# peter-seres/python-ray-tracer

Measured on AMD Instinct MI355X. Metric: Mrays/sec + frame time (ms) at 1920x1080, 8 spheres, depth=3, higher is better.
Workload: dtype f64

## Files before the change

### python-ray-tracer_amd/csrc/rt_device.h

```cpp
#pragma once
#include <hip/hip_runtime.h>
#include <stdint.h>

#pragma clang fp contract(off)

#ifndef RT_FAST_DIVSQRT
#define RT_FAST_DIVSQRT 1
#endif
#ifndef RT_FAST_NORMALIZE
#define RT_FAST_NORMALIZE 1
#endif
#ifndef RT_W_PARK
#define RT_W_PARK 7
#endif
#ifndef RT_W_AAPARK
#define RT_W_AAPARK 7
#endif
#ifndef RT_W_LANES
#define RT_W_LANES 4
#endif

namespace rt {

constexpr int TILE = 8;
// ... 151 lines not shown

enum { HIT_NONE = 0, HIT_SPHERE = 1, HIT_PLANE = 2 };

typedef __attribute__((address_space(3))) double lds_f64;
__device__ __forceinline__ unsigned fresh_lane()
{
    unsigned l;
    asm volatile("v_mbcnt_lo_u32_b32 %0, -1, 0\n\tv_mbcnt_hi_u32_b32 %0, -1, %0" : "=v"(l));
    return l;
}
template <bool PARK, int WGT, bool REMAT = false> struct Park3 {
    volatile lds_f64 *p;
    volatile lds_f64 *sbase;
    V3 v;
    __device__ __forceinline__ Park3(double *base, int slot, int wave = 0)
        : p(REMAT ? nullptr : (volatile lds_f64 *)base + slot * 3 * WGT + threadIdx.x),
          sbase(REMAT ? (volatile lds_f64 *)base + slot * 3 * WGT + wave * 64 : nullptr), v{0.0, 0.0, 0.0} {}
    __device__ __forceinline__ volatile lds_f64 *at() const { if constexpr (REMAT) return sbase + fresh_lane(); else return p; }
    __device__ __forceinline__ void set(const V3 &a)
    {
        if constexpr (PARK) { volatile lds_f64 *q = at(); q[0] = a.x; q[WGT] = a.y; q[2 * WGT] = a.z; } else v = a;
    }
    __device__ __forceinline__ V3 get() const
    {
        if constexpr (PARK) { volatile lds_f64 *q = at(); return V3{q[0], q[WGT], q[2 * WGT]}; } else return v;
    }
};

enum class Family { PLAIN, MAT, REFR, SCAT, SOFT, LENS, LENS_SOFT };
constexpr int FAMILIES = 7;
__host__ __device__ constexpr bool has_mat(Family f) { return f != Family::PLAIN; }
__host__ __device__ constexpr bool has_refr(Family f) { return f >= Family::REFR; }
__host__ __device__ constexpr bool has_scat(Family f) { return f >= Family::SCAT; }
__host__ __device__ constexpr bool has_soft(Family f) { return f == Family::SOFT || f == Family::LENS_SOFT; }
__host__ __device__ constexpr bool has_lens(Family f) { return f >= Family::LENS; }
__host__ __device__ constexpr int table_cols(Family f) { return has_scat(f) ? 6 : (has_refr(f) ? 5 : 3); }

template <Family F, int WSLOT, bool FRESH> struct MatState {
    static constexpr bool mat = true, refr = has_refr(F), scat = has_scat(F), soft = has_soft(F), lens = has_lens(F);
    static constexpr int COLS = table_cols(F);
    unsigned tab;
    unsigned ids;
    int nsh;
    enum { W = 0, LAMB = 1, REFL = 2, QX = 3, QY = 4, QZ = 5, ETA = 6, ROUGH = 7, KEY = 8, LKEY = 9 };
    template <int WGT, int k> __device__ __forceinline__ volatile lds_f64 *at(const double *acc, int wave) const
    {
        if constexpr (FRESH) return (volatile lds_f64 *)acc + (WSLOT + k) * WGT + wave * 64 + fresh_lane();
        else return (volatile lds_f64 *)acc + (WSLOT + k) * WGT + threadIdx.x;
    }
    __device__ __forceinline__ volatile const lds_f64 *entry(int slot) const
    {
        unsigned t = tab, i = ids;
        asm volatile("" : "+s"(t), "+s"(i));
        typedef __attribute__((address_space(3))) const int lds_ci32;
        const int m = ((lds_ci32 *)(size_t)i)[slot];
        return (volatile const lds_f64 *)(size_t)t + COLS * m;
    }
};
template <int WSLOT, bool FRESH> struct MatState<Family::PLAIN, WSLOT, FRESH> {
    static constexpr bool mat = false, refr = false, scat = false, soft = false, lens = false;
};

constexpr float CULL_K_ANCHOR = 0x1p-19f * 1.0001f;
constexpr float CULL_K_ORIGIN = 0x1p-18f;
constexpr float CULL_K_S = 0x1p-21f;
constexpr float CULL_K_FLOOR = 0x1p-40f;

extern __shared__ double lds_raw[];

struct Lds {
    __device__ __forceinline__ const double *recs() const { return lds_raw; }
    const float *sph32;
    const float *tab;
    const float *csph32;
    const float *ctab;
    const float *cbox;
    const float *gbox;
    const float *gtab;
    const float *col32;
    int NC;
    int wave;
    bool pairs;
    bool groups;
#ifdef RT_REGION_STATS
    unsigned *reg;
#endif
    double *acc;
};

#ifdef RT_REGION_STATS
__device__ __forceinline__ void region_mark(unsigned *reg, int id)
{
    volatile unsigned *r = reg + (threadIdx.x >> 6) * 32;
    const unsigned now = (unsigned)__builtin_amdgcn_s_memtime();
    const unsigned last = r[31], c = r[30];
    r[id + c] = r[id + c] + (now - last);
    r[31] = now;
}
#define RT_MARK(id) region_mark(lds.reg, id)
#else
#define RT_MARK(id)
#endif

struct RayF {
    F3 o, R;
    float mgq, esq;
};

__device__ __forceinline__ RayF make_rayf_dir(const V3 &R)
{
    RayF q;
    q.o = F3{0.0f, 0.0f, 0.0f};
    q.R = F3{(float)R.x, (float)R.y, (float)R.z};
    q.mgq = 0.0f; q.esq = 0.0f;
    return q;
}
__device__ __forceinline__ void add_origin(RayF &q, const V3 &o, float extent2)
{
    q.o = F3{(float)o.x, (float)o.y, (float)o.z};
    const float oo = __builtin_fmaf(q.o.z, q.o.z, __builtin_fmaf(q.o.y, q.o.y, q.o.x * q.o.x));
    q.mgq = __builtin_fmaf(CULL_K_ORIGIN, oo, CULL_K_FLOOR * (oo + extent2));
    q.esq = __builtin_fmaf(CULL_K_S, oo, CULL_K_S);
}

__device__ __forceinline__ float anchored_tau(double ll, double r2, float floor_anch)
{
    const double W = ((ll - r2) - (ll + r2) * (double)CULL_K_ANCHOR) - (double)floor_anch;
    if (!(W > 0.0)) return 0.0f;
    return (float)(__builtin_sqrt(W) * (1.0 - 0x1p-20));
}

typedef float f4 __attribute__((ext_vector_type(4)));
typedef __attribute__((address_space(3))) const f4 lds_cf4;
__device__ __forceinline__ lds_cf4 *pin_lds(const float *generic)
{
    unsigned a = (unsigned)(size_t)(__attribute__((address_space(3))) const float *)generic;
    asm volatile("" : "+v"(a));
    return (lds_cf4 *)(size_t)a;
}

__device__ __forceinline__ bool cull_anchored(const f4 e, const RayF &q)
{
    const float s = __builtin_fmaf(e[2], q.R.z, __builtin_fmaf(e[1], q.R.y, e[0] * q.R.x));
    return __builtin_fabsf(s) < e[3];
}

__device__ __forceinline__ bool cull_origin(const f4 c, const RayF &q)
{
    const float lx = q.o.x - c[0], ly = q.o.y - c[1], lz = q.o.z - c[2];
    const float s = __builtin_fmaf(lz, q.R.z, __builtin_fmaf(ly, q.R.y, lx * q.R.x));
    const float ll = __builtin_fmaf(lz, lz, __builtin_fmaf(ly, ly, lx * lx));
    const float cc = ll - c[3];
    const float D = __builtin_fmaf(s, s, -cc);
    const float mg = __builtin_fmaf(CULL_K_ORIGIN, ll + c[3], q.mgq);
    const float es = __builtin_fmaf(CULL_K_S, ll, q.esq);
    return (bool)((int)(D < -mg) | ((int)(s > es) & (int)(cc > mg)));
}

typedef unsigned long long lanemask;
__device__ __forceinline__ lanemask m_nlt_abs(float a, float b)
{
    lanemask m; asm volatile("v_cmp_nlt_f32_e64 %0, |%1|, %2" : "=s"(m) : "v"(a), "v"(b)); return m;
}
__device__ __forceinline__ lanemask m_nlt_neg(float a, float b)
{
    lanemask m; asm volatile("v_cmp_nlt_f32_e64 %0, %1, -%2" : "=s"(m) : "v"(a), "v"(b)); return m;
// ... 85 lines not shown
            open = m_nlt_abs(sd, e[3]);
        } else {
            const float lx = q.o.x - e[0], ly = q.o.y - e[1], lz = q.o.z - e[2];
            const float sd = __builtin_fmaf(lz, q.R.z, __builtin_fmaf(ly, q.R.y, lx * q.R.x));
            const float ll = __builtin_fmaf(lz, lz, __builtin_fmaf(ly, ly, lx * lx));
            const float cc = ll - e[3];
            const float D = __builtin_fmaf(sd, sd, -cc);
            const float mg = __builtin_fmaf(CULL_K_ORIGIN, ll + e[3], q.mgq);
            const float es = __builtin_fmaf(CULL_K_S, ll, q.esq);
            open = m_nlt_neg(D, mg) & (m_ngt(sd, es) | m_ngt(cc, mg));
        }
        if constexpr (SELF) open &= m_ne(jsel, u);
        acc = push_any(acc, open);
    }
    return acc;
}

template <bool ANCH, bool SELF>
__device__ __forceinline__ unsigned long long cull_mask_t(const Lds &lds, int S, int anchor, int k0, int n,
                                                          const RayF &q, int selfj)
{
    unsigned long long mask = 0ull;
    const int Sp = padS(S, lds.NC);
    lds_cf4 *sbase = pin_lds(ANCH ? lds.tab + ((size_t)anchor * Sp + k0) * CULL_STRIDE : lds.sph32 + 4 * k0);
    if (lds.NC > 0) {
        const int NCp = pad4(lds.NC), c0 = k0 / CLUSTER, nc = (n + CLUSTER - 1) / CLUSTER;
        if (ANCH && lds.groups) {
            static_assert(CLUSTER * SUPER == 64, "a 64-sphere chunk is one group of clusters");
            const f4 ge = *pin_lds(lds.gtab + ((size_t)anchor * pad4(supers(lds.NC)) + (k0 >> 6)) * CULL_STRIDE);
            const float gs = __builtin_fmaf(ge[2], q.R.z, __builtin_fmaf(ge[1], q.R.y, ge[0] * q.R.x));
            if (m_nlt_abs(gs, ge[3]) == 0ull) return 0ull;
        }
        lds_cf4 *cbase = pin_lds(ANCH ? lds.ctab + ((size_t)anchor * NCp + c0) * CULL_STRIDE : lds.csph32 + 4 * c0);
        unsigned cm = 0;
        for (int j = 0; j < nc; j += 4) cm |= (lds.pairs ? cull4<ANCH, false, true>(cbase + j, q, -1, 0u) : cull4<ANCH, false, false>(cbase + j, q, -1, 0u)) << j;
        while (cm) {
            const int c = __builtin_ctz(cm);
            cm &= cm - 1u;
            const int jb = c * CLUSTER;
            const unsigned hi = lds.pairs ? cull4<ANCH, SELF, true>(sbase + jb + 4, q, selfj - jb - 4, 0u) : cull4<ANCH, SELF, false>(sbase + jb + 4, q, selfj - jb - 4, 0u);
            const unsigned lohi = lds.pairs ? cull4<ANCH, SELF, true>(sbase + jb, q, selfj - jb, hi) : cull4<ANCH, SELF, false>(sbase + jb, q, selfj - jb, hi);
            mask |= (unsigned long long)lohi << jb;
        }
    } else {
        const int npad = pad4(n);
        for (int j = 0; j < npad; j += 4) mask |= (unsigned long long)(lds.pairs ? cull4<ANCH, SELF, true>(sbase + j, q, selfj - j, 0u) : cull4<ANCH, SELF, false>(sbase + j, q, selfj - j, 0u)) << j;
    }
    return mask;
}

__device__ __forceinline__ unsigned long long cull_mask(const Lds &lds, int S, int anchor, int k0, int n,
                                                        const V3 &o, const V3 &R, float extent2, int self)
{
    RayF q = make_rayf_dir(R);
    if (anchor >= 0) {
        const bool cand = self >= k0 && self < k0 + n;
        if (__builtin_amdgcn_ballot_w64(cand) != 0ull) {
            add_origin(q, o, extent2);
            const float *cs = lds.sph32 + 4 * self;
            const bool self_culled = cand ? cull_origin(f4{cs[0], cs[1], cs[2], cs[3]}, q) : false;
            if (__builtin_amdgcn_ballot_w64(self_culled) != 0ull)
                return cull_mask_t<true, true>(lds, S, anchor, k0, n, q, self_culled ? self - k0 : -1);
        }
        return cull_mask_t<true, false>(lds, S, anchor, k0, n, q, -1);
    }
    add_origin(q, o, extent2);
    return cull_mask_t<false, false>(lds, S, anchor, k0, n, q, -1);
}


__device__ __forceinline__ int opaque(int x)
{
    asm volatile("" : "+s"(x));
    return x;
}

__device__ __forceinline__ int plane_code(const KParams &p, int k)
{
    unsigned c = p.plane_codes;
    asm volatile("" : "+s"(c));
    return k < 4 ? (int)(signed char)(c >> (8 * k)) : 0;
}

__device__ __forceinline__ void plane_den_num(const double *__restrict__ g, int code, const V3 &o, const V3 &d, double &den, double &num)
{
    if (code == 0) {
        const V3 n{g[3], g[4], g[5]};
        den = dot3(d, n);
        const V3 LP{g[0] - o.x, g[1] - o.y, g[2] - o.z};
        num = dot3(LP, n);
    } else {
        const int a = code < 0 ? -code : code;
        double dc, lp;
        if (a == 1)      { dc = d.x; lp = g[0] - o.x; }
        else if (a == 2) { dc = d.y; lp = g[1] - o.y; }
        else             { dc = d.z; lp = g[2] - o.z; }
        if (code > 0) { den = dc; num = lp; } else { den = -dc; num = -lp; }
    }
}

struct SphHot { double x, y, z, r2; };
template <bool F32> __device__ __forceinline__ SphHot sphere_hot(const Lds &lds, int k)
{
    if constexpr (F32) {
        const f4 c = *(lds_cf4 *)(size_t)(unsigned)(size_t)(__attribute__((address_space(3))) const float *)(lds.sph32 + 4 * k);
        return SphHot{(double)c[0], (double)c[1], (double)c[2], (double)c[3]};
    } else {
        const double *g = lds.recs() + k * SPH_STRIDE;
        return SphHot{g[0], g[1], g[2], g[3]};
    }
}
template <bool F32> __device__ __forceinline__ double sphere_orig(const Lds &lds, const KParams &p, int k)
{
    if constexpr (F32) return p.scene[(size_t)k * SPH_STRIDE + 7]; else return lds.recs()[k * SPH_STRIDE + 7];
}

template <bool F32>
__device__ __forceinline__ void sphere_closest(const Lds &lds, const KParams &p, int k, const V3 &o, const V3 &R, double a,
                                               double &bestn, int &bidx)
{
    const SphHot g = sphere_hot<F32>(lds, k);
    const V3 Lv{o.x - g.x, o.y - g.y, o.z - g.z};
    const double s = dot3(Lv, R);
    const double cc = dot3(Lv, Lv) - g.r2;
    const double D = s * s - a * cc;
    if (D >= 0.0 && !(s >= 0.0 && cc >= 0.0)) {
        const double q = sqrt_inrange(D);
        double n = -s - q;
        if (!(n > 0.0)) n = -s + q;
        if (n > 0.0) {
            bool take = n < bestn;
            const bool close = __builtin_fabs(n - bestn) < bestn * 0x1p-50;
            if (__builtin_amdgcn_ballot_w64(close) != 0ull) {
                if (close) {
                    const double tq = n / a, tb = bestn / a;
                    take = tq < tb || (tq == tb && sphere_orig<F32>(lds, p, k) < sphere_orig<F32>(lds, p, bidx));
                }
            }
            if (take) { bestn = n; bidx = k; }
        }
    }
}

template <bool F32>
__device__ __forceinline__ bool sphere_any(const Lds &lds, int k, const V3 &o, const V3 &R, double a, bool a_sane)
{
    const SphHot g = sphere_hot<F32>(lds, k);
    const V3 Lv{o.x - g.x, o.y - g.y, o.z - g.z};
    const double s = dot3(Lv, R);
    const double cc = dot3(Lv, Lv) - g.r2;
    const double D = s * s - a * cc;
    if (D >= 0.0 && !(s >= 0.0 && cc >= 0.0)) {
        if (s < 0.0 && -s < 499.0 && D < 249001.0 && a_sane) return true;
        const double q = __builtin_sqrt(D);
        double n = -s - q;
        if (!(n > 0.0)) n = -s + q;
        if (n > 0.0) {
            const double t = n / a;
            if (999.0 > t && t > 0.0) return true;
        }
    }
    return false;
}


template <bool ANCH>
__device__ __forceinline__ bool lane_open(const f4 e, const RayF &q)
{
    if constexpr (ANCH) {
        const float sd = __builtin_fmaf(e[2], q.R.z, __builtin_fmaf(e[1], q.R.y, e[0] * q.R.x));
        return !(__builtin_fabsf(sd) < e[3]);
    } else return !cull_origin(e, q);
}
__device__ __forceinline__ lds_cf4 *lds_f4(const float *generic)
{
    return (lds_cf4 *)(size_t)(unsigned)(size_t)(__attribute__((address_space(3))) const float *)generic;
}

template <bool ANCH>
__device__ __forceinline__ unsigned lane_cluster_bits(const Lds &lds, int anchor, int cb, int nc, const RayF &q, float extent2)
{
    unsigned cm = 0u;
    if constexpr (ANCH) {
        const int NCp = pad4(lds.NC), NGp = pad4(supers(lds.NC));
        lds_cf4 *base = pin_lds(lds.ctab + ((size_t)anchor * NCp + cb) * CULL_STRIDE);
        lds_cf4 *gbase = pin_lds(lds.gtab + ((size_t)anchor * NGp + cb / SUPER) * CULL_STRIDE);
        for (int c0 = 0; c0 < nc; c0 += SUPER) {
            if (__builtin_amdgcn_ballot_w64(lane_open<true>(gbase[c0 / SUPER], q)) == 0ull) continue;
            const int c1 = c0 + SUPER < nc ? c0 + SUPER : nc;
            for (int c = c0; c < c1; c += 4) {
#pragma unroll
                for (int u = 0; u < 4; ++u) {
                    asm volatile("" ::: "memory");
                    const f4 e = base[c + u];
                    cm |= lane_open<true>(e, q) ? (1u << (c + u)) : 0u;
                }
            }
        }
    } else {
        const RayBox rb = make_raybox(q, extent2);
        lds_cf4 *base = pin_lds(lds.cbox + (size_t)cb * BOX_STRIDE);
        lds_cf4 *gbase = pin_lds(lds.gbox + (size_t)(cb / SUPER) * BOX_STRIDE);
        static_assert(SUPER == 8, "a group's clusters are one byte of the mask");
        for (int c0 = 0; c0 < nc; c0 += SUPER) {
            const bool gopen = box_open(gbase[2 * (c0 / SUPER)], gbase[2 * (c0 / SUPER) + 1], rb) || !rb.sane;
            if (__builtin_amdgcn_ballot_w64(gopen) == 0ull) continue;
            const int c1 = c0 + SUPER < nc ? c0 + SUPER : nc;
            for (int c = c0; c < c1; c += 2) {
#pragma unroll
                for (int u = 0; u < 2; ++u) {
                    asm volatile("" ::: "memory");
                    const f4 lo = base[2 * (c + u)], hi = base[2 * (c + u) + 1];
                    cm |= box_open(lo, hi, rb) ? (1u << (c + u)) : 0u;
                }
            }
        }
        if (!rb.sane) cm = ~0u;
    }
    return cm & (nc >= 32 ? ~0u : ((1u << nc) - 1u));
}

template <bool ANCH>
__device__ __forceinline__ unsigned lane_sphere_bits(const Lds &lds, int S, int anchor, int kb, const RayF &q)
{
    const int Sp = padS(S, lds.NC);
    lds_cf4 *sb = lds_f4(ANCH ? lds.tab + ((size_t)anchor * Sp + kb) * CULL_STRIDE : lds.sph32 + 4 * kb);
    unsigned sm = 0u;
#pragma unroll
    for (int j = 0; j < CLUSTER; ++j) sm |= lane_open<ANCH>(sb[j], q) ? (1u << j) : 0u;
    const int nv = S - kb;
    return nv >= CLUSTER ? sm : (sm & ((1u << nv) - 1u));
}

#ifdef RT_LANE_STATS
__device__ __forceinline__ void lane_stats(const KParams &p, int base, unsigned v)
{
    if (!p.tile_cycles) return;
    unsigned mx = v, sum = v;
    for (int d = 32; d >= 1; d >>= 1) { const unsigned m2 = __shfl_xor(mx, d), s2 = __shfl_xor(sum, d); mx = m2 > mx ? m2 : mx; sum += s2; }
    if ((threadIdx.x & 63) == __builtin_ctzll(__builtin_amdgcn_ballot_w64(true))) {
        unsigned *c = p.tile_cycles + p.ntiles + base;
        atomicAdd(c + 0, 1u); atomicAdd(c + 1, mx); atomicAdd(c + 2, (sum + 63u) >> 6); atomicAdd(c + 3, sum);
    }
}
#endif
// ... 47 lines not shown
        if (__builtin_amdgcn_ballot_w64(self >= 0) != 0ull) {
            add_origin(q, o, p.extent2);
            if (self >= 0) { const float *cs = lds.sph32 + 4 * self; self_culled = cull_origin(f4{cs[0], cs[1], cs[2], cs[3]}, q); }
        }
    } else add_origin(q, o, p.extent2);
    bool occ = false;
    for (int cb = 0; cb < lds.NC; cb += 32) {
        if (cb > 0 && __builtin_amdgcn_ballot_w64(!occ) == 0ull) break;
        const int nc = lds.NC - cb < 32 ? lds.NC - cb : 32;
        unsigned cm = lane_cluster_bits<ANCH>(lds, anchor, cb, nc, q, p.extent2);
        RT_MARK(7);
        if (occ) cm = 0u;
#ifdef RT_LANE_STATS
        lane_stats(p, 8, __builtin_popcount(cm));
#endif
        while (__builtin_amdgcn_ballot_w64(cm != 0u) != 0ull) {
#ifdef RT_LANE_STATS
            unsigned smc = 0;
#endif
            if (cm != 0u) {
                const int kb = (cb + __builtin_ctz(cm)) * CLUSTER;
                cm &= cm - 1u;
                unsigned sm = lane_sphere_bits<ANCH>(lds, p.S, anchor, kb, q);
                if (self_culled && self >= kb && self < kb + CLUSTER) sm &= ~(1u << (self - kb));
#ifdef RT_LANE_STATS
                smc = __builtin_popcount(sm);
#endif
                while (__builtin_amdgcn_ballot_w64(sm != 0u) != 0ull) {
                    if (sm != 0u) {
                        const int k = kb + __builtin_ctz(sm);
                        sm &= sm - 1u;
                        if (sphere_any<true>(lds, k, o, R, a, a_sane)) { occ = true; sm = 0u; cm = 0u; }
                    }
                }
            }
#ifdef RT_LANE_STATS
            lane_stats(p, 12, smc);
#endif
        }
        RT_MARK(8);
    }
    return occ;
}

template <int MODE>
__device__ __forceinline__ void closest_hit(const Lds &lds, const KParams &p, const V3 &o, const V3 &d, int anchor,
                                            double &t_out, int &idx_out, int &type_out)
{
    const int P = opaque(p.P);
    const int S = p.S;
    const V3 R = renormalize_unit(d);
    const double a = dot3(R, R);
    RT_MARK(0);
    const int canchor = (opaque(p.anchors) > 0) ? anchor : -1;
    double bestn = __builtin_inf();
    int bidx = -1;
    constexpr bool F32 = MODE >= 1;
    if (MODE >= 2 && lds.NC > 0 && (canchor < 0 || p.lanes_primary)) {
        if (canchor >= 0) lanes_closest<true>(lds, p, canchor, o, R, a, bestn, bidx);
        else lanes_closest<false>(lds, p, -1, o, R, a, bestn, bidx);
    } else
    for (int k0 = 0; k0 < S; k0 += 64) {
      const int n = (S - k0 < 64) ? S - k0 : 64;
      unsigned long long mask = cull_mask(lds, S, canchor, k0, n, o, R, p.extent2, -1);
      mask &= (n == 64) ? ~0ull : ((1ull << n) - 1ull);
      RT_MARK(1);
      while (mask) {
        const int k = k0 + __builtin_ctzll(mask);
        mask &= mask - 1ull;
        sphere_closest<F32>(lds, p, k, o, R, a, bestn, bidx);
      }
      RT_MARK(2);
    }
    double best = 999.0;
    int idx = -1, type = HIT_NONE;
    if (bidx >= 0) {
        const double t = div_inrange(bestn, a);
        if (best > t && t > 0.0) { best = t; idx = bidx; type = HIT_SPHERE; }
    }
    const double *pl = lds.recs() + (F32 ? 0 : opaque(p.S) * SPH_STRIDE);
    for (int k = 0; k < P; ++k) {
        const double *g = pl + k * PL_STRIDE;
        double den, num;
        plane_den_num(g, plane_code(p, k), o, d, den, num);
        if (!(__builtin_fabs(den) < 0.001)) {
            const double t = div_inrange(num, den);
            if (best > t && t > 0.0) { best = t; idx = k; type = HIT_PLANE; }
        }
    }
    t_out = best; idx_out = idx; type_out = type;
    RT_MARK(3);
}

template <int MODE>
__device__ __forceinline__ bool any_hit(const Lds &lds, const KParams &p, const V3 &o, const V3 &d, int anchor, int self, bool lanes = true)
{
    const int P = opaque(p.P);
    const int S = p.S;
    const V3 R = renormalize_unit(d);
    const double a = dot3(R, R);
    RT_MARK(6);
    const bool a_sane = (a > 0.999999 && a < 1.000001);
    bool occ = false;
    const int canchor = (opaque(p.anchors) > 0) ? anchor : -1;
    if (MODE >= 2 && lds.NC > 0 && lanes) {
        occ = (canchor >= 0) ? lanes_any<true>(lds, p, canchor, o, R, a, self) : lanes_any<false>(lds, p, -1, o, R, a, self);
    } else
    for (int k0 = 0; k0 < S; k0 += 64) {
      if (k0 > 0 && __builtin_amdgcn_ballot_w64(!occ) == 0ull) break;
      const int n = (S - k0 < 64) ? S - k0 : 64;
      unsigned long long mask = cull_mask(lds, S, canchor, k0, n, o, R, p.extent2, self);
      mask &= (n == 64) ? ~0ull : ((1ull << n) - 1ull);
      RT_MARK(7);
      while (mask) {
        const int k = k0 + __builtin_ctzll(mask);
        mask &= mask - 1ull;
        if (!occ) occ = sphere_any<(MODE >= 1)>(lds, k, o, R, a, a_sane);
        if (mask && __builtin_amdgcn_ballot_w64(!occ) == 0ull) break;
      }
      RT_MARK(8);
    }
    const double *pl = lds.recs() + (MODE >= 1 ? 0 : opaque(p.S) * SPH_STRIDE);
    for (int k = 0; k < P; ++k) {
        if (!occ) {
            const double *g = pl + k * PL_STRIDE;
            double den, num;
            plane_den_num(g, plane_code(p, k), o, d, den, num);
            if (!(__builtin_fabs(den) < 0.001)) {
                const double an = __builtin_fabs(num), ad = __builtin_fabs(den);
                const bool same_sign = (num > 0.0 && den > 0.0) || (num < 0.0 && den < 0.0);
                if (same_sign) {
                    if (an < 998.0 * ad) occ = true;
                    else if (!(an > 1000.0 * ad)) { const double t = num / den; if (999.0 > t && t > 0.0) occ = true; }
                }
            }
        }
    }
    RT_MARK(9);
    return occ;
}

template <bool COUNT> struct RayCount {
    __device__ __forceinline__ void closest(bool) {}
    __device__ __forceinline__ void hit(bool) {}
    __device__ __forceinline__ void shadow(bool, bool) {}
};
template <> struct RayCount<true> {
    unsigned n_closest = 0, n_issued = 0, n_skipped = 0, n_hit = 0;
    __device__ __forceinline__ void closest(bool alive) { n_closest += alive ? 1u : 0u; }
    __device__ __forceinline__ void hit(bool alive) { n_hit += alive ? 1u : 0u; }
    __device__ __forceinline__ void shadow(bool alive, bool traced) { n_issued += (alive && traced) ? 1u : 0u; n_skipped += (alive && !traced) ? 1u : 0u; }
};

__device__ __forceinline__ unsigned scatter_key(unsigned x, unsigned y, unsigned s, unsigned seed)
{
    unsigned h = (seed ^ 0x5CA77E12u) ^ 0x9E3779B9u;
    h = (h ^ x) * 0x85EBCA6Bu; h ^= h >> 13;
    h = (h ^ y) * 0xC2B2AE35u; h ^= h >> 16;
    return h ^ (s << 9);
}
__device__ __forceinline__ unsigned scatter_hash(unsigned key, unsigned t)
{
    unsigned h = (key ^ t) * 0x27D4EB2Fu; h ^= h >> 15;
    h *= 0x165667B1u; h ^= h >> 13;
    return h;
}

__device__ __forceinline__ unsigned soft_key(unsigned x, unsigned y, unsigned s, unsigned seed)
{
    unsigned h = (seed ^ 0x50F7117Eu) ^ 0x9E3779B9u;
    h = (h ^ x) * 0x85EBCA6Bu; h ^= h >> 13;
    h = (h ^ y) * 0xC2B2AE35u; h ^= h >> 16;
    return h ^ (s << 20);
}

__device__ __forceinline__ V3 soft_light_point(unsigned key, const double *g)
{
#pragma unroll 1
    for (int j = 0; j < 8; ++j) {
// ... 431 lines not shown
        }
        b[3] = 0.0f; b[7] = 0.0f;
    }
    __syncthreads();
    for (int g = threadIdx.x; g < supers(p.NC); g += TABLE_THREADS) {
        float *b = out + tl.gbox + (size_t)g * BOX_STRIDE;
        for (int i = 0; i < 3; ++i) { b[i] = __builtin_inff(); b[4 + i] = -__builtin_inff(); }
        for (int c = g * SUPER; c < (g + 1) * SUPER && c < p.NC; ++c)
            for (int i = 0; i < 3; ++i) {
                b[i] = __builtin_fminf(b[i], cbox[(size_t)c * BOX_STRIDE + i]);
                b[4 + i] = __builtin_fmaxf(b[4 + i], cbox[(size_t)c * BOX_STRIDE + 4 + i]);
            }
        b[3] = 0.0f; b[7] = 0.0f;
    }
    const int NG = supers(p.NC), NGp = pad4(NG);
    const double *gr = cl + (size_t)p.NC * CL_STRIDE;
    for (int e = threadIdx.x; e < p.anchors * NGp; e += TABLE_THREADS) {
        const int a = e / NGp, g = e - a * NGp;
        float *t = out + tl.gtab + (size_t)e * CULL_STRIDE;
        if (g >= NG) { t[0] = t[1] = t[2] = 0.0f; t[3] = -NINF; continue; }
        const double *c = gr + g * CL_STRIDE;
        const double ax = a ? lt[(a - 1) * LT_STRIDE + 0] : p.cam_o[0];
        const double ay = a ? lt[(a - 1) * LT_STRIDE + 1] : p.cam_o[1];
        const double az = a ? lt[(a - 1) * LT_STRIDE + 2] : p.cam_o[2];
        const double lx = ax - c[0], ly = ay - c[1], lz = az - c[2];
        const double ll = lx * lx + ly * ly + lz * lz;
        t[0] = (float)lx; t[1] = (float)ly; t[2] = (float)lz;
        t[3] = anchored_tau(ll, c[3], p.floor_anch);
    }
}

template <Family F, int WSLOT, bool FRESH>
__device__ __forceinline__ MatState<F, WSLOT, FRESH> mat_state(double *matl, int M, int nsh = 1)
{
    typedef __attribute__((address_space(3))) double lds_d;
    typedef MatState<F, WSLOT, FRESH> MS;
    if constexpr (MS::mat) return MS{(unsigned)(size_t)(lds_d *)(matl + 1), (unsigned)(size_t)(lds_d *)(matl + 1 + MS::COLS * M), nsh};
    else return {};
}

template <bool AA, bool PARK, int WPW, bool COUNT = false, bool LAT = false, int MODE = 0, Family F = Family::PLAIN>
__global__ __launch_bounds__(64 * WPW, MODE >= 2 ? RT_W_LANES : (AA ? (PARK ? RT_W_AAPARK : 4) : (PARK ? RT_W_PARK : 5))) void render_kernel(const KParams p)
{
    constexpr int WG_THREADS = 64 * WPW, WAVES_PER_WG = WPW;
    constexpr bool M2 = MODE >= 2;
    constexpr bool NOREC = MODE >= 1;
    constexpr bool MAT = has_mat(F), SCAT = has_scat(F), SOFT = has_soft(F), LENS = has_lens(F);
    const int nrec = (int)lds_doubles(NOREC ? 0 : p.S, p.P, p.L);
    const double *rec_src = p.scene + (NOREC ? (size_t)p.S * SPH_STRIDE : 0);
    double *accum = lds_raw + nrec;
    int *offw = reinterpret_cast<int *>(accum + lds_slots(AA, PARK, M2, F) * WG_THREADS);
    float *sph32 = reinterpret_cast<float *>(offw + lds_offset_words(PARK, WG_THREADS));
    const TableLayout tl = table_layout(p.S, p.NC, p.anchors, p.P);
    const bool LANES = MODE >= 2 && p.anchors > 0;
    float *tab = sph32 + tl.tab;
    float *csph32 = LANES ? nullptr : sph32 + tl.csph32;
    float *ctab = sph32 + tl.ctab;
    float *cbox = sph32 + tl.cbox;
    const size_t ntab = MODE == 1 ? tl.total_col : (LANES ? tl.total_lanes : tl.total);
    unsigned *wgstat = reinterpret_cast<unsigned *>(sph32 + ntab);
    if (threadIdx.x == 0) { wgstat[0] = 0u; wgstat[1] = 0u; }
    {
        for (int i = threadIdx.x; i < nrec; i += WG_THREADS) lds_raw[i] = rec_src[i];
        const int nf4 = (int)(ntab / 4);
        const f4 *src = reinterpret_cast<const f4 *>(p.ftab);
        f4 *dst = reinterpret_cast<f4 *>(sph32);
        for (int i = threadIdx.x; i < nf4; i += WG_THREADS) dst[i] = src[i];
    }
#ifdef RT_REGION_STATS
    double *matl = reinterpret_cast<double *>(wgstat + 4 + WPW * 32);
#else
    double *matl = reinterpret_cast<double *>(wgstat + 4);
#endif
    int nmat = 0, nsh = 1;
    if constexpr (MAT) {
        const double *msrc = p.scene + (LENS ? (size_t)p.lens.mat : mat_offset(p.S, p.P, p.L, p.NC));
        nmat = (int)msrc[0];
        const int nm = (int)mat_doubles(nmat, p.S, p.P, F);
        for (int i = threadIdx.x; i < nm; i += WG_THREADS) matl[i] = msrc[i];
        if constexpr (SOFT) nsh = (int)msrc[nm - 1];
    }
    __syncthreads();
#ifdef RT_REGION_STATS
    const Lds lds{sph32, tab, csph32, ctab, cbox, sph32 + tl.gbox, sph32 + tl.gtab, MODE == 1 ? sph32 + tl.col32 : nullptr, WPW == 2 ? 0 : p.NC, __builtin_amdgcn_readfirstlane((int)(threadIdx.x >> 6)), MODE < 2, MODE >= 2, wgstat + 4, accum};
    for (int i = threadIdx.x & 63; i < 32; i += 64) lds.reg[(threadIdx.x >> 6) * 32 + i] = 0u;
    if ((threadIdx.x & 63) == 0) lds.reg[(threadIdx.x >> 6) * 32 + 31] = (unsigned)__builtin_amdgcn_s_memtime();
#else
    const Lds lds{sph32, tab, csph32, ctab, cbox, sph32 + tl.gbox, sph32 + tl.gtab, MODE == 1 ? sph32 + tl.col32 : nullptr, WPW == 2 ? 0 : p.NC, __builtin_amdgcn_readfirstlane((int)(threadIdx.x >> 6)), MODE < 2, MODE >= 2, accum};
#endif

    const int wave = threadIdx.x >> 6, lane = threadIdx.x & 63;
    int bid = (int)blockIdx.x;
    const unsigned *ord = p.order;
    if (p.nframes > 1) {
        const int frame = div_by(bid, p.bpf, p.bpf_magic, p.bpf_shift);
        bid -= frame * p.bpf;
        if (ord && frame < p.nframes - 1) ord += p.seq_offset;
    }
    const bool by_tile = WPW >= TILE_ORDER_MIN_WPW && p.order_tiles;
    const int block = by_tile ? bid : (ord ? (int)ord[bid] : bid);
    const int wave_u = __builtin_amdgcn_readfirstlane(wave);
    const int tile_v = by_tile ? (ord ? (int)ord[bid * WAVES_PER_WG + wave_u] : bid * WAVES_PER_WG + wave_u) : block * WAVES_PER_WG + wave;
    const int tile = WPW >= TILE_ORDER_MIN_WPW ? __builtin_amdgcn_readfirstlane(tile_v) : tile_v;
    if (tile >= p.ntiles) return;
    const unsigned long long t_begin = (p.tile_cycles || p.cost) ? __builtin_amdgcn_s_memtime() : 0ull;
    const int tx = div_by(tile, p.tiles_y, p.tiles_y_magic, p.tiles_y_shift), ty = tile - tx * p.tiles_y;
    const int x = p.x0 + tx * TILE + (lane >> 3);
    const int y = ty * TILE + (lane & 7);
    bool inb = (x < p.x1) && (y < p.h);
    if constexpr (LAT) inb = inb && ((((x | y) & 1) == 0) || (x >= 1 && x <= p.w - 2 && y >= 1 && y <= p.h - 2));
    const int xc = inb ? x : p.x0, yc = inb ? y : 0;
    typedef __attribute__((address_space(3))) int lds_i32;
    constexpr bool OFF_REMAT = PARK && MODE == 3;
    volatile lds_i32 *offp = OFF_REMAT ? nullptr : (volatile lds_i32 *)offw + threadIdx.x;
    if constexpr (PARK && !OFF_REMAT) *offp = inb ? (x - p.x0) * p.h + y : -1;

    const V3 o{p.cam_o[0], p.cam_o[1], p.cam_o[2]};
    RayCount<COUNT> cnt;
    constexpr int WSLOT = lds_slots(AA, PARK, M2, Family::PLAIN);
    auto ms = mat_state<F, WSLOT, !PARK || MODE == 3>(matl, nmat, nsh);
    const unsigned sseed = SCAT ? p.seed : 0u;
    double R, G, B;
    if constexpr (!AA) {
        unsigned key = 0u, lkey = 0u;
        if constexpr (SCAT) key = LAT ? scatter_key((unsigned)xc, (unsigned)yc, 0u, sseed) : scatter_key(2u * xc, 2u * yc, 0u, sseed);
        if constexpr (SOFT) lkey = LAT ? soft_key((unsigned)xc, (unsigned)yc, 0u, sseed) : soft_key(2u * xc, 2u * yc, 0u, sseed);
        const V3 P0 = LAT ? lattice_P(p, xc, yc) : pixel_P(p, xc, yc);
        V3 ro = o, rd;
        if constexpr (LENS) lens_ray(p, LAT ? (unsigned)xc : 2u * xc, LAT ? (unsigned)yc : 2u * yc, 0u, P0, ro, rd);
        else rd = primary_dir(p, P0);
        const V3 c = sample<PARK, WG_THREADS, COUNT, MODE, decltype(ms)>(lds, p, inb, ro, rd, cnt, ms, key, lkey);
        R = c.x; G = c.y; B = c.z;
    } else {
        const bool stoch = (p.aa == 2);
        const bool interior = !stoch && inb && x >= 1 && x <= p.w - 2 && y >= 1 && y <= p.h - 2;
        const int ntaps = stoch ? p.spp : ((__builtin_amdgcn_ballot_w64(interior) != 0ull) ? 9 : 1);
        constexpr unsigned NBX = 0x8858u, NBY = 0x0A25u;
        Park3<PARK && !M2, WG_THREADS> taps(lds.acc, 2);
#pragma unroll 1
        for (int tap = 0; tap < ntaps; ++tap) {
            const V3 Pp = pixel_P(p, xc, yc);
            V3 Pt = Pp;
            unsigned key = 0u, lkey = 0u;
            unsigned lx = 2u * xc, ly = 2u * yc;
            if constexpr (SCAT) key = scatter_key(2u * xc, 2u * yc, stoch ? (unsigned)tap : 0u, sseed);
            if constexpr (SOFT) lkey = soft_key(2u * xc, 2u * yc, stoch ? (unsigned)tap : 0u, sseed);
            if (stoch) {
                const unsigned hh = jitter_hash((unsigned)xc, (unsigned)yc, (unsigned)tap, p.seed);
                const double u = (double)(hh & 0xFFFFu) * 0x1p-16 + (0x1p-17 - 0.5);
                const double v = (double)(hh >> 16) * 0x1p-16 + (0x1p-17 - 0.5);
                Pt = V3{Pp.x, Pp.y + u * p.dy, Pp.z + v * p.dz};
            } else if (tap) {
                const int k = tap - 1;
                const int ddx = (int)((NBX >> (2 * k)) & 3u) - 1, ddy = (int)((NBY >> (2 * k)) & 3u) - 1;
                const V3 Pn = pixel_P(p, interior ? x + ddx : xc, interior ? y + ddy : yc);
                Pt = V3{0.5 * Pp.x + 0.5 * Pn.x, 0.5 * Pp.y + 0.5 * Pn.y, 0.5 * Pp.z + 0.5 * Pn.z};
                if constexpr (SCAT) key = scatter_key((unsigned)(2 * xc + ddx), (unsigned)(2 * yc + ddy), 0u, sseed);
                if constexpr (SOFT) lkey = soft_key((unsigned)(2 * xc + ddx), (unsigned)(2 * yc + ddy), 0u, sseed);
                if constexpr (LENS) { lx = (unsigned)(2 * xc + ddx); ly = (unsigned)(2 * yc + ddy); }
            }
            V3 ro = o, rd;
            if constexpr (LENS) lens_ray(p, lx, ly, stoch ? (unsigned)tap : 0u, Pt, ro, rd);
            else rd = primary_dir(p, Pt);
            const V3 s = sample<PARK, WG_THREADS, COUNT, MODE, decltype(ms)>(lds, p, (tap && !stoch) ? interior : inb, ro, rd, cnt, ms, key, lkey);
            if (tap == 0) taps.set(s);
            else if (stoch) { const V3 a = taps.get(); taps.set(V3{a.x + s.x, a.y + s.y, a.z + s.z}); }
            else if (interior) { const V3 a = taps.get(); taps.set(V3{a.x + s.x, a.y + s.z, a.z + s.y}); }
        }
        { const V3 a = taps.get(); R = a.x; G = a.y; B = a.z; }
        if (stoch) { const double n = (double)p.spp; R = R / n; G = G / n; B = B / n; }
        else if (interior) { R = R / 9; G = G / 9; B = B / 9; }
// ... 172 lines not shown
```

Before: 200,500.

## Add wave-mask based shadow any-hit path with plane sign test

Adds a shadow-ray any-hit routine that keeps occupancy as 64-bit wave ballot masks instead of per-lane booleans. Sphere and plane tests classify lanes into certain-hit and edge cases with compares and sign checks, and only edge lanes run the sqrt or divide. The goal is to cut divergent sqrt/divide work and exit early once every live lane is occluded. It is enabled through a new trim flag only for the two-wave-per-workgroup, no-material variant, and it also skips negating plane den/num in closest-hit when trim is set. That skip looks safe only because t = num/den does not change sign, and the extra ballots add scalar overhead.

New measurement: 210,200 (median of 6 runs). +4.8%, better.

```diff
diff --git a/python-ray-tracer_amd/csrc/rt_device.h b/python-ray-tracer_amd/csrc/rt_device.h
--- a/python-ray-tracer_amd/csrc/rt_device.h
+++ b/python-ray-tracer_amd/csrc/rt_device.h
@@ -257,6 +257,7 @@
     int wave;
     bool pairs;
     bool groups;
+    bool trim;
 #ifdef RT_REGION_STATS
     unsigned *reg;
 #endif
@@ -508,7 +509,8 @@
     return k < 4 ? (int)(signed char)(c >> (8 * k)) : 0;
 }
 
-__device__ __forceinline__ void plane_den_num(const double *__restrict__ g, int code, const V3 &o, const V3 &d, double &den, double &num)
+__device__ __forceinline__ void plane_den_num(const double *__restrict__ g, int code, const V3 &o, const V3 &d, double &den, double &num,
+                                              bool no_negate = false)
 {
     if (code == 0) {
         const V3 n{g[3], g[4], g[5]};
@@ -521,7 +523,7 @@
         if (a == 1)      { dc = d.x; lp = g[0] - o.x; }
         else if (a == 2) { dc = d.y; lp = g[1] - o.y; }
         else             { dc = d.z; lp = g[2] - o.z; }
-        if (code > 0) { den = dc; num = lp; } else { den = -dc; num = -lp; }
+        if (code > 0 || no_negate) { den = dc; num = lp; } else { den = -dc; num = -lp; }
     }
 }
 
@@ -587,6 +589,41 @@
         }
     }
     return false;
+}
+
+__device__ __forceinline__ bool lane_of(lanemask m)
+{
+    unsigned x; asm("v_cndmask_b32_e64 %0, 0, 1, %1" : "=v"(x) : "s"(m)); return x != 0u;
+}
+__device__ __forceinline__ lanemask lanes_where(bool c) { return __builtin_amdgcn_ballot_w64(c); }
+
+template <bool F32>
+__device__ __forceinline__ lanemask sphere_any_mask(const Lds &lds, int k, const V3 &o, const V3 &R, double a, lanemask a_sane)
+{
+    const SphHot g = sphere_hot<F32>(lds, k);
+    const V3 Lv{o.x - g.x, o.y - g.y, o.z - g.z};
+    const double s = dot3(Lv, R);
+    const double cc = dot3(Lv, Lv) - g.r2;
+    const double D = s * s - a * cc;
+    const lanemask dpos = lanes_where(D >= 0.0), sneg = lanes_where(s < 0.0);
+    const lanemask cand = dpos & (sneg | lanes_where(!(cc >= 0.0)));
+    const lanemask fast = dpos & sneg & lanes_where(-s < 499.0) & lanes_where(D < 249001.0) & a_sane;
+    lanemask hit = fast;
+    const lanemask slow = cand & ~fast;
+    if (slow != 0ull) {
+        bool h = false;
+        if (lane_of(slow)) {
+            const double q = __builtin_sqrt(D);
+            double n = -s - q;
+            if (!(n > 0.0)) n = -s + q;
+            if (n > 0.0) {
+                const double t = n / a;
+                h = 999.0 > t && t > 0.0;
+            }
+        }
+        hit |= lanes_where(h);
+    }
+    return hit;
 }
 
 
@@ -800,7 +837,7 @@
     for (int k = 0; k < P; ++k) {
         const double *g = pl + k * PL_STRIDE;
         double den, num;
-        plane_den_num(g, plane_code(p, k), o, d, den, num);
+        plane_den_num(g, plane_code(p, k), o, d, den, num, lds.trim);
         if (!(__builtin_fabs(den) < 0.001)) {
             const double t = div_inrange(num, den);
             if (best > t && t > 0.0) { best = t; idx = k; type = HIT_PLANE; }
@@ -810,9 +847,58 @@
     RT_MARK(3);
 }
 
+__device__ __forceinline__ bool any_hit_masks(const Lds &lds, const KParams &p, const V3 &o, const V3 &d, int anchor, int self)
+{
+    const int P = opaque(p.P);
+    const int S = p.S;
+    const V3 R = renormalize_unit(d);
+    const double a = dot3(R, R);
+    RT_MARK(6);
+    const int canchor = (opaque(p.anchors) > 0) ? anchor : -1;
+    const lanemask live = lanes_where(true);
+    const lanemask a_sane = lanes_where(a > 0.999999) & lanes_where(a < 1.000001);
+    lanemask occ = 0ull;
+    for (int k0 = 0; k0 < S; k0 += 64) {
+      if (k0 > 0 && (live & ~occ) == 0ull) break;
+      const int n = (S - k0 < 64) ? S - k0 : 64;
+      unsigned long long mask = cull_mask(lds, S, canchor, k0, n, o, R, p.extent2, self);
+      mask &= (n == 64) ? ~0ull : ((1ull << n) - 1ull);
+      RT_MARK(7);
+      while (mask) {
+        const int k = k0 + __builtin_ctzll(mask);
+        mask &= mask - 1ull;
+        occ |= sphere_any_mask<false>(lds, k, o, R, a, a_sane);
+        if (mask && (live & ~occ) == 0ull) break;
+      }
+      RT_MARK(8);
+    }
+    const double *pl = lds.recs() + opaque(p.S) * SPH_STRIDE;
+    for (int k = 0; k < P; ++k) {
+        if ((live & ~occ) == 0ull) break;
+        const double *g = pl + k * PL_STRIDE;
+        double den, num;
+        plane_den_num(g, plane_code(p, k), o, d, den, num, true);
+        const double an = __builtin_fabs(num), ad = __builtin_fabs(den);
+        int sx = (int)(__builtin_bit_cast(unsigned long long, num) >> 32) ^ (int)(__builtin_bit_cast(unsigned long long, den) >> 32);
+        asm("" : "+v"(sx));
+        const lanemask ahead = lanes_where(!(ad < 0.001)) & lanes_where(sx >= 0) & lanes_where(an > 0.0);
+        const lanemask sure = lanes_where(an < 998.0 * ad);
+        occ |= ahead & sure;
+        const lanemask edge = ahead & ~sure & ~occ;
+        if (edge != 0ull) {
+            bool h = false;
+            if (lane_of(edge) && !(an > 1000.0 * ad)) { const double t = num / den; h = 999.0 > t && t > 0.0; }
+            occ |= lanes_where(h);
+        }
+    }
+    RT_MARK(9);
+    return lane_of(occ);
+}
+
 template <int MODE>
 __device__ __forceinline__ bool any_hit(const Lds &lds, const KParams &p, const V3 &o, const V3 &d, int anchor, int self, bool lanes = true)
 {
+    if (MODE == 0 && lds.trim) return any_hit_masks(lds, p, o, d, anchor, self);
     const int P = opaque(p.P);
     const int S = p.S;
     const V3 R = renormalize_unit(d);
@@ -1410,11 +1496,11 @@
     }
     __syncthreads();
 #ifdef RT_REGION_STATS
-    const Lds lds{sph32, tab, csph32, ctab, cbox, sph32 + tl.gbox, sph32 + tl.gtab, MODE == 1 ? sph32 + tl.col32 : nullptr, WPW == 2 ? 0 : p.NC, __builtin_amdgcn_readfirstlane((int)(threadIdx.x >> 6)), MODE < 2, MODE >= 2, wgstat + 4, accum};
+    const Lds lds{sph32, tab, csph32, ctab, cbox, sph32 + tl.gbox, sph32 + tl.gtab, MODE == 1 ? sph32 + tl.col32 : nullptr, WPW == 2 ? 0 : p.NC, __builtin_amdgcn_readfirstlane((int)(threadIdx.x >> 6)), MODE < 2, MODE >= 2, WPW == 2 && !MAT, wgstat + 4, accum};
     for (int i = threadIdx.x & 63; i < 32; i += 64) lds.reg[(threadIdx.x >> 6) * 32 + i] = 0u;
     if ((threadIdx.x & 63) == 0) lds.reg[(threadIdx.x >> 6) * 32 + 31] = (unsigned)__builtin_amdgcn_s_memtime();
 #else
-    const Lds lds{sph32, tab, csph32, ctab, cbox, sph32 + tl.gbox, sph32 + tl.gtab, MODE == 1 ? sph32 + tl.col32 : nullptr, WPW == 2 ? 0 : p.NC, __builtin_amdgcn_readfirstlane((int)(threadIdx.x >> 6)), MODE < 2, MODE >= 2, accum};
+    const Lds lds{sph32, tab, csph32, ctab, cbox, sph32 + tl.gbox, sph32 + tl.gtab, MODE == 1 ? sph32 + tl.col32 : nullptr, WPW == 2 ? 0 : p.NC, __builtin_amdgcn_readfirstlane((int)(threadIdx.x >> 6)), MODE < 2, MODE >= 2, WPW == 2 && !MAT, accum};
 #endif
 
     const int wave = threadIdx.x >> 6, lane = threadIdx.x & 63;
```
